# czbiohub-sf/yogo

Measured on AMD Instinct MI355X. Metric: training images/sec (772x1032 gray), higher is better.
Workload: dtype bf16; 1 GPU; BASELINE configs[2]: full train step (fwd+loss+bwd+clamp+AdamW), base_model, 772x1032x1 uint8, 7 classes; per_gpu_batch=128, global_batch=128, parallelism=dp1

## Files before the change

include/yogo_hip.h:

```cpp
#ifndef YOGO_HIP_H
#define YOGO_HIP_H

#include <stddef.h>

#ifdef __cplusplus
extern "C" {
#endif

typedef void* yogo_stream_t;

const char* yogo_hip_last_error(void);
int yogo_hip_abi_version(void);
int yogo_hip_launch_log(int enable);
int yogo_hip_launch_log_read(char* buf, size_t cap, size_t* needed);


int yogo_conv_packed_bytes(int Cin, int Cout, int ksize, int stride, int mode, size_t* bytes);
int yogo_conv_pack_f32(const float* w_oihw, float* packed, int Cin, int Cout, int ksize, int stride, int mode,
                       yogo_stream_t stream);
int yogo_conv2d_fwd_stats_shape(int B, int Cin, int Cout, int IH, int IW, int ksize, int stride, int* rows, int* mpad);
int yogo_conv2d_fwd_f32(const float* in, const float* packed, const float* bias, float* out, float* out_pre,
                        const float* chan_scale, float* stats_part, int B, int Cin, int Cout, int IH, int IW, int ksize,
                        int stride, int act, yogo_stream_t stream);
int yogo_conv2d_dgrad_f32(const float* dy, const float* packed_dgrad, float* dx, const float* act_ref, int ref_act,
// ... 45 lines not shown

int yogo_format_preds_workspace_bytes(int B, int Sy, int Sx, size_t* bytes);
int yogo_format_preds_batched(const float* pred, float* out_rows, long long* out_cells, int* out_count, void* workspace,
                              int B, int P, int Sy, int Sx, int cap, double obj_thresh, double iou_thresh, int box_format,
                              double min_class_confidence_threshold, yogo_stream_t stream);
int yogo_decode_format_preds_batched(const float* raw, const float* cxs, const float* cys, float* out_rows, long long* out_cells,
                                     int* out_count, void* workspace, int B, int P, int Sy, int Sx, int cap, float anchor_w,
                                     float anchor_h, float width_multiplier, float height_multiplier, int inference,
                                     double obj_thresh, double iou_thresh, int box_format, double min_class_confidence_threshold,
                                     yogo_stream_t stream);
int yogo_head1x1_decode_fwd_bf16(const void* x, const void* packed, const float* bias, float* out, const float* cxs, const float* cys,
                                 int B, int Cin, int P, int Sy, int Sx, float anchor_w, float anchor_h, float width_multiplier,
                                 float height_multiplier, int inference, yogo_stream_t stream);

int yogo_match_workspace_bytes(int B, int Sy, int Sx, int cap, size_t* bytes);
int yogo_match_preds_labels_batched(const float* rows, const int* counts, const float* labels, int* meta, int* pair_label,
                                    int* pair_pred, int* un_label, int* un_pred, float* lab_out, void* workspace, int B, int P, int Sy,
                                    int Sx, int cap, yogo_stream_t stream);
int yogo_match_gather(const float* rows, const float* lab_out, const int* meta, const int* pair_label, const int* pair_pred,
                      const int* un_label, const int* un_pred, float* preds, float* labels, float* missed, float* extra, int B, int P,
                      int cap, long long K, long long Km, long long Ke, yogo_stream_t stream);
int yogo_metrics_state_layout(int C, int T, int nbins, long long* offsets);
int yogo_metrics_accumulate(const float* rows, const float* lab_out, const int* meta, const int* pair_label, const int* pair_pred,
                            const int* un_label, const int* un_pred, const double* roc_thresholds, int T, const double* cal_edges,
                            int nbins, long long* acc, double* bin_conf, double* partial, float* map_rows, long long map_cap, int B,
                            int P, int cap, yogo_stream_t stream);

int yogo_pred_sink_state_layout(int C, long long* offsets);
int yogo_pred_sink_workspace_bytes(int B, size_t* bytes);
int yogo_pred_sink_append(const float* rows, const int* counts, int B, int cap, int P, int mode, int count_classes,
                          long long first_img_id, int img_h, int img_w, long long* state, float* arena, long long arena_cap,
                          int* img_counts, long long img_cap, void* workspace, yogo_stream_t stream);
int yogo_pred_text_bound(long long n_records, long long images, int P, size_t* text_bytes, size_t* workspace_bytes);
int yogo_pred_text_format(const float* records, long long n, int P, const int* img_counts, long long images, char* text,
                          long long text_cap, long long* img_offsets, long long* total, void* workspace, yogo_stream_t stream);

int yogo_bf16_channel_blocks(int C);
int yogo_conv_bf16_packed_bytes(int Cin, int Cout, int ksize, int mode, size_t* bytes);
int yogo_conv_bf16_pack(const float* w_oihw, const float* scale, void* packed, int Cin, int Cout, int ksize, int mode,
                        yogo_stream_t stream);
int yogo_conv2d_fwd_bf16_stats_shape(int B, int Cin, int Cout, int IH, int IW, int ksize, int stride, int* rows, int* mpad);
int yogo_conv2d_fwd_bf16(const void* in, const void* packed, const float* bias, void* out, float* out_f32,
                         const float* chan_scale, float* stats_part, int B, int Cin, int Cout, int IH, int IW, int ksize,
                         int stride, int act, yogo_stream_t stream);
int yogo_conv2d_fwd_bf16_pre(const void* in, const void* packed, const float* bias, void* out, void* out_pre,
                             const float* chan_scale, int B, int Cin, int Cout, int IH, int IW, int ksize, int stride, int act,
                             yogo_stream_t stream);
int yogo_conv_bf16_pack_blocks(int Cin, int Cout, int ksize, int mode, int* blocks);
int yogo_conv_bf16_pack_multi(const void* table, int n, int total_blocks, yogo_stream_t stream);
int yogo_bf16_signs_bytes(int B, int C, int H, int W, size_t* bytes);
int yogo_conv2d_fwd_bf16_signs(const void* in, const void* packed, const float* bias, void* out, void* signs,
                               const float* chan_scale, int B, int Cin, int Cout, int IH, int IW, int ksize, int stride, int act,
                               yogo_stream_t stream);
int yogo_conv2d_dgrad_bf16_signs(const void* dy, const void* packed_dgrad, void* dx, const void* signs,
                                 const float* chan_scale, int B, int Cin, int Cout, int IH, int IW, int ksize, int stride,
                                 yogo_stream_t stream);
int yogo_conv2d_dgrad_bf16(const void* dy, const void* packed_dgrad, void* dx, const void* act_ref, int ref_act,
                           const float* chan_scale, int B, int Cin, int Cout, int IH, int IW, int ksize, int stride,
                           yogo_stream_t stream);
int yogo_conv2d_wgrad_bf16in(const void* x, const void* g, float* dw, float* db, void* workspace, int B, int Cin, int Cout,
                             int IH, int IW, int ksize, int stride, float clip, yogo_stream_t stream);
int yogo_conv2d_wgrad_bf16_workspace_bytes(int B, int Cin, int Cout, int IH, int IW, int ksize, int stride, size_t* bytes);
int yogo_conv2d_wgrad_bf16(const void* x, const void* g, float* dw, float* db, void* workspace, int B, int Cin, int Cout,
                           int IH, int IW, int ksize, int stride, float clip, yogo_stream_t stream);
int yogo_wgrad_reduce_queue_create(void** queue_out);
int yogo_wgrad_reduce_queue_destroy(void* queue);
int yogo_wgrad_reduce_queue_reset(void* queue);
int yogo_wgrad_reduce_flush(void* queue, yogo_stream_t stream);
int yogo_conv2d_wgrad_bf16_deferred(const void* x, const void* g, float* dw, float* db, void* workspace, int B, int Cin, int Cout, int IH,
                                    int IW, int ks, int stride, float clip, void* queue, yogo_stream_t stream);
int yogo_conv_first_fwd_bf16(const void* in, int in_dtype, const float* w, const float* bias, void* out, int B, int Cin,
                             int Cout, int IH, int IW, int stride, int act, yogo_stream_t stream);
int yogo_conv_first_fwd_train_bf16(const void* in, int in_dtype, const float* w, const float* bias, void* out_bf16,
                                   const float* chan_scale, float* stats_part, int B, int Cin, int Cout, int IH, int IW,
                                   int stride, int act, yogo_stream_t stream);
int yogo_conv_first_wgrad_bf16g(const void* in, int in_dtype, const void* dy_bf16, float* part, int B, int Cin, int Cout,
                                int IH, int IW, int stride, yogo_stream_t stream);
int yogo_conv_first_bn_wgrad_cols(int Cin, int Cout, int* cols);
int yogo_conv_first_bn_wgrad_bf16(const void* in, int in_dtype, const void* g, const void* z, const float* mean,
                                  const float* invstd, const float* gamma, const float* beta, float* part, int B, int Cin,
                                  int Cout, int IH, int IW, int stride, int act, yogo_stream_t stream);
int yogo_conv_first_bn_wgrad_finalize(const float* sums, const float* mean, const float* invstd, const float* gamma,
                                      const float* w_oihw, float* dw, float* dgamma, float* dbeta, int B, int Cin, int Cout,
                                      int IH, int IW, int stride, int training, float clip, yogo_stream_t stream);
int yogo_bn_apply_act_bf16(const void* z, void* y, const float* mean, const float* invstd_or_var, int stat_is_var, float eps,
                           const float* gamma, const float* beta, int B, int C, int HW, int act, yogo_stream_t stream);
int yogo_bn_bwd_bf16_rows(int B, int HW, int* rows);
int yogo_bn_stats_bf16(const void* z, float* part, int B, int C, int HW, yogo_stream_t stream);
int yogo_bn_bwd_bf16(const void* g, const void* z, void* dz, const float* mean, const float* invstd, const float* gamma,
                     const float* beta, int act, float* dgamma, float* dbeta, float* part, float* sums, int B, int C, int HW,
                     int training, float clip, yogo_stream_t stream);
int yogo_bn_bwd_bf16_head(const void* gh, const float* head_w, int P, const void* z, void* dz, const float* mean, const float* invstd,
                          const float* gamma, const float* beta, int act, float* dgamma, float* dbeta, float* part, float* sums, int B,
                          int C, int HW, int training, float clip, yogo_stream_t stream);
int yogo_nchw_f32_to_bf16_8c(const float* in, void* out, int B, int C, int HW, yogo_stream_t stream);
int yogo_bf16_8c_to_nchw_f32(const void* in, float* out, int B, int C, int HW, yogo_stream_t stream);

int yogo_conv_first_mfma_supported(int in_dtype, int Cin, int Cout, int IH, int IW, int stride);
int yogo_conv_first_mfma_stats_rows(int B, int IH, int IW, int* rows);
int yogo_conv_first_mfma(const void* in, const float* w, const float* bias, void* z, void* y, const float* mean,
                         const float* invstd, const float* gamma, const float* beta, float* stats_part, int B, int Cout, int IH,
                         int IW, int act, yogo_stream_t stream);

int yogo_conv_first_gram_rows(int B, int IH, int IW, int* rows);
int yogo_conv_first_gram(const void* in, void* part, double* gram, float* gram_f32, int B, int IH, int IW, yogo_stream_t stream);
int yogo_bn_stats_from_gram(const double* gram, const float* w, const float* bias, int Cout, long long count, float eps,
// ... 91 lines not shown
```

yogo_amd/csrc/conv_bf16.hip:

```cpp
#include "conv_bf16_plan.h"
#include "conv_bf16_ws.h"
#include "conv_bf16_ws16.h"
#include "conv_bf16_ws3.h"
#include "plan_switches.h"

#ifdef YOGO_DIAG
static int g_diag_dbg = 0, g_diag_nodma = 0;
static unsigned long long* g_diag_stamps = nullptr;
static size_t g_diag_stamps_bytes = 0;
extern "C" int yogo_diag_conv_bf16(int dbg_bits, int no_dma, void* stamps, size_t stamps_bytes) {
  g_diag_dbg = dbg_bits; g_diag_nodma = no_dma;
  g_diag_stamps = reinterpret_cast<unsigned long long*>(stamps); g_diag_stamps_bytes = stamps_bytes;
  return YOGO_OK;
}
template <typename Q>
void bf_diag_persistent(Q* q, hipStream_t stream) {
  q->dbg = g_diag_dbg;
  q->stamps = (g_diag_stamps != nullptr && g_diag_stamps_bytes >= 512 * 128) ? g_diag_stamps : nullptr;
  if (q->stamps) (void)hipMemsetAsync(g_diag_stamps, 0, 512 * 128, stream);
}
#else
template <typename Q>
void bf_diag_persistent(Q*, hipStream_t) {}
#endif
// ... 183 lines not shown
  BfTiledPlan pl;
  if (int e = bf_plan_tiled(r, &pl)) return e;
  return launch_conv_bf16_tiled(r, pl, stream);
}

}

extern "C" int yogo_conv2d_fwd_bf16_stats_shape(int B, int Cin, int Cout, int IH, int IW, int ks, int stride, int* rows, int* mpad) {
  ConvBf16Request r;
  if (int e = bf_request(B, Cin, Cout, IH, IW, ks, stride, BF_FORWARD, &r)) return e;
  BfTiledPlan pl;
  if (int e = bf_plan_tiled(r, &pl)) return e;
  if (rows) *rows = pl.rows;
  if (mpad) *mpad = pl.mpad;
  return YOGO_OK;
}

extern "C" int yogo_conv2d_fwd_bf16(const void* in, const void* packed, const float* bias, void* out, float* out_f32,
                                    const float* chan_scale, float* stats_part, int B, int Cin, int Cout, int IH, int IW,
                                    int ks, int stride, int act, hipStream_t stream) {
  YOGO_CHECK_ARG(in && packed && (out || out_f32), "conv2d_fwd_bf16: null pointer");
  ConvBf16Request r;
  if (int e = bf_request(B, Cin, Cout, IH, IW, ks, stride, BF_FORWARD, &r)) return e;
  r.in = in; r.packed = packed; r.bias = bias; r.out = out; r.out_f32 = out_f32; r.chan_scale = chan_scale; r.stats_part = stats_part; r.act = act;
  return launch_conv_bf16(r, stream);
}

extern "C" int yogo_conv2d_fwd_bf16_pre(const void* in, const void* packed, const float* bias, void* out, void* out_pre,
                                        const float* chan_scale, int B, int Cin, int Cout, int IH, int IW, int ks, int stride,
                                        int act, hipStream_t stream) {
  YOGO_CHECK_ARG(in && packed && out && out_pre, "conv2d_fwd_bf16_pre: null pointer");
  ConvBf16Request r;
  if (int e = bf_request(B, Cin, Cout, IH, IW, ks, stride, BF_FORWARD, &r)) return e;
  r.in = in; r.packed = packed; r.bias = bias; r.out = out; r.out_pre = out_pre; r.chan_scale = chan_scale; r.act = act;
  return launch_conv_bf16(r, stream);
}

extern "C" int yogo_bf16_signs_bytes(int B, int C, int H, int W, size_t* bytes) {
  YOGO_CHECK_ARG(bytes && B >= 0 && C > 0 && H > 0 && W > 0, "bf16_signs_bytes: bad arguments");
  *bytes = (size_t)B * H * W * (bf_mpad_of(C) / 8);
  return YOGO_OK;
}

extern "C" int yogo_conv2d_fwd_bf16_signs(const void* in, const void* packed, const float* bias, void* out, void* signs,
                                          const float* chan_scale, int B, int Cin, int Cout, int IH, int IW, int ks, int stride,
                                          int act, hipStream_t stream) {
  YOGO_CHECK_ARG(in && packed && out && signs, "conv2d_fwd_bf16_signs: null pointer");
  ConvBf16Request r;
  if (int e = bf_request(B, Cin, Cout, IH, IW, ks, stride, BF_FORWARD, &r)) return e;
  r.in = in; r.packed = packed; r.bias = bias; r.out = out; r.signs = signs; r.chan_scale = chan_scale; r.act = act;
  return launch_conv_bf16(r, stream);
}

extern "C" int yogo_conv2d_dgrad_bf16_signs(const void* dy, const void* packed_dgrad, void* dx, const void* signs,
                                            const float* chan_scale, int B, int Cin, int Cout, int IH, int IW, int ks, int stride,
                                            hipStream_t stream) {
  YOGO_CHECK_ARG(dy && packed_dgrad && dx && signs, "conv2d_dgrad_bf16_signs: null pointer");
  ConvBf16Request r;
  if (int e = bf_request(B, Cin, Cout, IH, IW, ks, stride, BF_DGRAD, &r)) return e;
  r.in = dy; r.packed = packed_dgrad; r.out = dx; r.ref_act = ACT_LEAKY; r.signs = const_cast<void*>(signs); r.signs_read = true; r.chan_scale = chan_scale;
  return launch_conv_bf16(r, stream);
}

extern "C" int yogo_conv2d_dgrad_bf16(const void* dy, const void* packed_dgrad, void* dx, const void* act_ref, int ref_act,
                                      const float* chan_scale, int B, int Cin, int Cout, int IH, int IW, int ks, int stride,
                                      hipStream_t stream) {
  YOGO_CHECK_ARG(dy && packed_dgrad && dx, "conv2d_dgrad_bf16: null pointer");
  ConvBf16Request r;
  if (int e = bf_request(B, Cin, Cout, IH, IW, ks, stride, BF_DGRAD, &r)) return e;
  r.in = dy; r.packed = packed_dgrad; r.out = dx; r.act_ref = act_ref; r.ref_act = ref_act; r.chan_scale = chan_scale;
  return launch_conv_bf16(r, stream);
}
```

yogo_amd/csrc/conv_bf16_plan.h:

```cpp
#pragma once
#include "common.h"

#define BF_LDS_BUDGET (80 * 1024)
#define BF_LDS_MAX (160 * 1024)

__host__ __device__ inline int bf_pick_mw(int M) { return M <= 32 ? 1 : (M <= 64 ? 2 : 4); }
__host__ __device__ inline int bf_kb_of(int K) { return (K + 15) / 16 * 2; }
__host__ __device__ inline int bf_mpad_of(int M) { const int t = 32 * bf_pick_mw(M); return (M + t - 1) / t * t; }

struct ConvBf16Request {
  const void* in;
  const void* packed;
  const float* bias;
  void* out;
  float* out_f32;
  void* out_pre;
  const void* act_ref;
  int ref_act;
  void* signs;
  bool signs_read;
  const float* chan_scale;
  float* stats_part;
  int B, K, M, IH, IW, OH, OW, ks, a, s2d, act;
#ifdef YOGO_DIAG
  int dbg;
  unsigned long long* stamps;
  size_t stamps_bytes;
#endif
};

struct BfTiling {
  int ncb, TW, tiles_per_band, CKb, rows_max, LW, ldsw_off, lds_dummy, lds_bytes, dma, ni_slots, n_slots, bufu;
};

struct BfTiledPlan {
  int MW, NW, NWV, PF;
  bool wide64;
  BfTiling tl;
  bool ring;
  int lean4, rowdma, lwp;
  int dma;
  bool use_pp;
  int ni_slots, n_slots, ldsw_off, bufu, bufs, lds_bytes;
  dim3 grid;
  int rows, mpad;
};

int launch_conv_bf16_tiled(const ConvBf16Request& r, const BfTiledPlan& pl, hipStream_t stream);
bool conv_bf16_s2d_direct_eligible(int K, int M, int OH, int OW, int B);
int launch_conv_bf16_s2d_direct(const void* in, const void* packed, void* out, const void* signs, const float* chan_scale, int B, int K, int M, int IH, int IW,
                                int OH, int OW, hipStream_t stream);
bool conv_bf16_staged_eligible(int K, int M, int stride, int IH, int IW, int OH, int OW, int B);
int launch_conv_bf16_staged(const void* in, const void* packed, const float* bias, void* out, void* signs, const float* chan_scale, int B, int K, int M, int IH,
                            int IW, int OH, int OW, int stride, int act, hipStream_t stream);
bool conv_bf16_head_fwd_eligible(int K, int M, int plane, int B);
int launch_conv_bf16_head_fwd(const void* in, const void* packed, const float* bias, float* out_f32, int B, int K, int M, int plane, hipStream_t stream);
```

yogo_amd/csrc/plan_switches.h:

```cpp
#pragma once

bool plan_ws();
int plan_ws16_mode();
bool plan_direct();
bool plan_staged();
bool plan_head();
bool plan_first_bn_wgrad_pairs();
bool plan_first_mfma_pairs();
bool plan_tiled_pp();
bool plan_tiled_ring();
bool plan_tiled_lean4();
bool plan_tiled_rowdma();
```

yogo_amd/csrc/plan_switches.hip:

```cpp
#include "common.h"
#include "plan_switches.h"

#ifndef BF_WS16_MODE
#define BF_WS16_MODE 1
#endif
#ifdef BF_NO_ROWDMA
#define BF_ROWDMA_DEFAULT false
#else
#define BF_ROWDMA_DEFAULT true
#endif

#define PLAN_HOOK_SWITCHES(X)                                                              \
  X(bool, plan_ws, true, yogo_hook_conv_bf16_persistent)                                   \
  X(int, plan_ws16_mode, BF_WS16_MODE, yogo_hook_conv_bf16_ws16)                           \
  X(bool, plan_direct, true, yogo_hook_conv_bf16_direct)                                   \
  X(bool, plan_staged, true, yogo_hook_conv_bf16_staged)                                   \
  X(bool, plan_head, true, yogo_hook_conv_bf16_head)                                       \
  X(bool, plan_first_bn_wgrad_pairs, true, yogo_hook_conv_first_bn_wgrad_pairs)            \
  X(bool, plan_first_mfma_pairs, true, yogo_hook_conv_first_mfma_pairs)
#define PLAN_DIAG_SWITCHES(X)                                                              \
  X(bool, plan_tiled_pp, true, yogo_diag_conv_bf16_pp)                                     \
  X(bool, plan_tiled_ring, true, yogo_diag_conv_bf16_ring)                                 \
  X(bool, plan_tiled_lean4, true, yogo_diag_conv_bf16_lean4)                               \
  X(bool, plan_tiled_rowdma, BF_ROWDMA_DEFAULT, yogo_diag_conv_bf16_rowdma)

#define PLAN_CONSTANT(T, NAME, DEFAULT, SETTER) \
  T NAME() { return DEFAULT; }
#define PLAN_VARIABLE(T, NAME, DEFAULT, SETTER)                                            \
  static T g_##NAME = DEFAULT;                                                             \
  T NAME() { return g_##NAME; }                                                            \
  extern "C" int SETTER(int v) { g_##NAME = static_cast<T>(v); return YOGO_OK; }

#if defined(YOGO_TEST_HOOKS) || defined(YOGO_DIAG)
PLAN_HOOK_SWITCHES(PLAN_VARIABLE)
#else
PLAN_HOOK_SWITCHES(PLAN_CONSTANT)
#endif
#ifdef YOGO_DIAG
PLAN_DIAG_SWITCHES(PLAN_VARIABLE)
#else
PLAN_DIAG_SWITCHES(PLAN_CONSTANT)
#endif
```

yogo_amd/engine.py:

```python
from __future__ import annotations

import threading
import weakref
from dataclasses import dataclass, field
from typing import Dict, List, Optional, Tuple

import torch
from torch import nn

from yogo_amd import _hip

ACT_NONE, ACT_LEAKY, ACT_SILU = 0, 1, 2


@dataclass
class Layer:
    conv: nn.Conv2d
    bn: Optional[nn.BatchNorm2d] = None
    act: int = ACT_NONE
    drop: Optional[nn.Dropout2d] = None

    @property
    def cin(self) -> int:
        return self.conv.in_channels
# ... 272 lines not shown
                          IW, L.s, st)
                red = torch.empty(L.cout, nj, dtype=torch.float32, device=dev)
                _hip.call("yogo_partials_reduce", part, rows, L.cout * nj, clip, red, st)
                dw.copy_(red[:, : nj - 1].reshape(dw.shape))
                if has_bias:
                    db = dst(L.conv.bias)
                    db.copy_(red[:, nj - 1])
                    grads[id(L.conv.bias)] = db
            else:
                wsb = _hip.query_size("yogo_conv2d_wgrad_workspace_bytes", B, L.cin, L.cout, IH, IW, L.k, L.s)
                ws = torch.empty(wsb // 4, dtype=torch.float32, device=dev)
                db = dst(L.conv.bias) if has_bias else None
                self._tick("wgrad", i, 2.0 * B * L.cout * L.cin * L.k * L.k * OH * OW)
                _hip.call("yogo_conv2d_wgrad_f32", S.x_in, g, dw, db, ws, B, L.cin, L.cout, IH, IW, L.k, L.s, clip, st)
                self._tock()
                if has_bias:
                    grads[id(L.conv.bias)] = db
            grads[id(L.conv.weight)] = dw
            if on_layer is not None:
                on_layer(i)
            if i > 0:
                Lp, Sp = self.layers[i - 1], saved[i - 1]
                ref_act = Lp.act
                if Lp.bn is not None:
                    act_ref, ref_act = None, ACT_NONE
                elif Lp.act == ACT_SILU:
                    act_ref = Sp.pre
                    if act_ref is None:
                        raise RuntimeError("yogo_amd: missing saved pre-activation for a SiLU block")
                elif Lp.act == ACT_LEAKY:
                    act_ref = Sp.y
                else:
                    act_ref = None
                dx = torch.empty(B, L.cin, IH, IW, dtype=torch.float32, device=dev)
                pk = self._packed(i, 1)
                mw_tag = 20 if L.s == 2 else (4 if L.cin > 64 else (2 if L.cin > 32 else 1))
                self._tick("dgrad", i, 2.0 * B * L.cout * L.cin * L.k * L.k * OH * OW, mw=mw_tag)
                _hip.call("yogo_conv2d_dgrad_f32", g, pk, dx, act_ref, ref_act, Sp.mask, B, L.cin, L.cout, IH, IW, L.k, L.s, st)
                self._tock()
                g = dx
        bb = self.backbone_ref()
        return [grads.get(id(p)) for p in bb.parameters()]



def _blocks(c: int) -> int:
    return ((c + 15) // 16) * 2


_FUSE_LAYER0_BWD = True
_L0_NO_Z = True
_WGRAD_DEFER_REDUCE = True
_L01_FUSE_BWD = True
_HEAD_BN_FUSE = True


def _packed_bf16(eng: Engine, i: int, mode: int) -> torch.Tensor:
    L = eng.layers[i]
    w = L.conv.weight
    key = (i, 10 + mode)
    buf = _pack_hit(eng, key, w)
    if buf is not None:
        return buf
    nbytes = _hip.query_size("yogo_conv_bf16_packed_bytes", L.cin, L.cout, L.k, mode)
    buf = torch.empty(nbytes, dtype=torch.uint8, device=w.device)
    _hip.call("yogo_conv_bf16_pack", _f32(w.detach()), None, buf, L.cin, L.cout, L.k, mode, _hip.stream_ptr())
    eng._pack[key] = (w._version, w.data_ptr(), buf)
    return buf


def _pack_all_bf16(eng: Engine) -> None:
    jobs = [(i, mode) for i in range(1, len(eng.layers)) for mode in (0, 2 if (eng.layers[i].s == 2 and eng.layers[i].k == 3) else 1)]
    ws = [eng.layers[i].conv.weight for i, _ in jobs]
    if any(w.dtype != torch.float32 or not w.is_contiguous() for w in ws) or not jobs:
        return
    if all(_pack_hit(eng, (i, 10 + m), w) is not None for (i, m), w in zip(jobs, ws)):
        return
    dev = ws[0].device
    key = tuple(w.data_ptr() for w in ws)
    st = eng._pack_multi
    if st is None or st[0] != key:
        bufs, rows, blk = [], [], 0
        for (i, mode), w in zip(jobs, ws):
            L = eng.layers[i]
            buf = torch.empty(_hip.query_size("yogo_conv_bf16_packed_bytes", L.cin, L.cout, L.k, mode), dtype=torch.uint8, device=dev)
            bufs.append(buf)
            rows.append([w.data_ptr(), 0, buf.data_ptr(), L.cin, L.cout, L.k, mode, blk])
            blk += _hip.query_ints("yogo_conv_bf16_pack_blocks", 1, L.cin, L.cout, L.k, mode)[0]
        st = (key, bufs, torch.tensor(rows, dtype=torch.int64, device=dev), blk)
        eng._pack_multi = st
    _, bufs, table, blk = st
    _hip.call("yogo_conv_bf16_pack_multi", table, len(jobs), blk, _hip.stream_ptr())
    for (i, mode), w, buf in zip(jobs, ws, bufs):
        eng._pack[(i, 10 + mode)] = (w._version, w.data_ptr(), buf)


def _dropout_masks(eng: Engine, B: int, dev) -> Dict[int, torch.Tensor]:
    act = [(i, float(L.drop.p)) for i, L in enumerate(eng.layers) if L.drop is not None and L.drop.training and L.drop.p > 0]
    if not act:
        return {}
    key = (B, tuple(act), str(dev))
    cached = eng._drop_consts
    if cached is None or cached[0] != key:
        sizes = [B * eng.layers[i].cout for i, _ in act]
        pvec = torch.cat([torch.full((n,), p, dtype=torch.float32) for n, (_, p) in zip(sizes, act)]).to(dev)
        cached = (key, sizes, pvec, 1.0 / (1.0 - pvec))
# ... 58 lines not shown


def _layer_fwd_bf16(eng: Engine, i: int, L: Layer, S: Saved, bias, bn_train: bool, last: bool, B: int, H: int, W: int, st) -> torch.Tensor:
    cur, mask, dev = S.x_in, S.mask, S.x_in.device
    OH, OW = L.out_hw(H, W)
    has_bn = L.bn is not None
    if last and (has_bn or mask is not None):
        raise RuntimeError("yogo_amd: BatchNorm / Dropout on the last layer is not supported by the bf16 path")
    fused_act = ACT_NONE if has_bn else L.act
    out8 = None if last else torch.empty(B, _blocks(L.cout), OH, OW, 8, dtype=torch.bfloat16, device=dev)
    out32 = torch.empty(B, L.cout, OH, OW, dtype=torch.float32, device=dev) if last else None
    stats = None
    rows = mpad = 0
    if i == 0:
        if bn_train:
            rows, mpad = _hip.query_ints("yogo_conv_first_stats_rows", 1, B, H, W, L.s)[0], L.cout
            stats = torch.empty(rows * mpad * 2, dtype=torch.float32, device=dev)
        _hip.call("yogo_conv_first_fwd_train_bf16", cur, 0 if cur.dtype == torch.uint8 else 1, _f32(L.conv.weight.detach()), bias,
                  out8, mask, stats, B, L.cin, L.cout, H, W, L.s, fused_act, st)
    else:
        pk = _packed_bf16(eng, i, 0)
        nbytes = B * (_blocks(L.cin) * 8 * H * W * 2 + (L.cout * OH * OW * 4 if last else _blocks(L.cout) * 8 * OH * OW * 2))
        eng._tick("fwd", i, 2.0 * B * L.cout * L.cin * L.k * L.k * OH * OW, mw=34 if (L.cout > 64 and L.s == 1) else (35 if (L.cout > 64 and L.cin > 64 and L.k == 3) else 30), nbytes=nbytes)
        if L.act == ACT_SILU and not has_bn:
            S.pre = torch.empty_like(out8)
            _hip.call("yogo_conv2d_fwd_bf16_pre", cur, pk, bias, out8, S.pre, mask, B, L.cin, L.cout, H, W, L.k, L.s, fused_act, st)
        elif L.act == ACT_LEAKY and not has_bn and not last:
            S.signs = torch.empty(_hip.query_size("yogo_bf16_signs_bytes", B, L.cout, OH, OW), dtype=torch.uint8, device=dev)
            _hip.call("yogo_conv2d_fwd_bf16_signs", cur, pk, bias, out8, S.signs, mask, B, L.cin, L.cout, H, W, L.k, L.s, fused_act, st)
        else:
            _hip.call("yogo_conv2d_fwd_bf16", cur, pk, bias, out8, out32, mask, None, B, L.cin, L.cout, H, W, L.k, L.s, fused_act, st)
        eng._tock()
    if not has_bn:
        S.y = out32 if last else out8
        return S.y
    bn = L.bn
    gamma, beta = _bn_affine(L, dev)
    y = torch.empty_like(out8)
    if bn_train:
        if i > 0:
            rows, mpad = _hip.query_ints("yogo_bn_bwd_bf16_rows", 1, B, OH * OW)[0], L.cout
            stats = torch.empty(rows * mpad * 2, dtype=torch.float32, device=dev)
            _hip.call("yogo_bn_stats_bf16", out8, stats, B, L.cout, OH * OW, st)
        mean, invstd = _bn_finalize(eng, L, "yogo_bn_finalize", stats, rows, mpad, count=B * OH * OW, dev=dev, st=st)
    else:
        invstd = torch.empty(L.cout, dtype=torch.float32, device=dev)
        _hip.call("yogo_bn_invstd", bn.running_var, float(bn.eps), invstd, L.cout, st)
        mean = bn.running_mean
    _hip.call("yogo_bn_apply_act_bf16", out8, y, mean, invstd, 0, float(bn.eps), gamma, beta, B, L.cout, OH * OW, L.act, st)
    S.mean, S.invstd, S.bn_train, S.z, S.y = mean, invstd, bn_train, out8, y
    return y


def forward_bf16_train(eng: Engine, x: torch.Tensor) -> Tuple[torch.Tensor, List[Saved]]:
    _check_bf16_train_input(eng, x)
    dev, st, B = x.device, _hip.stream_ptr(), x.shape[0]
    _pack_all_bf16(eng)
    masks = _dropout_masks(eng, B, dev)
    cur = x.contiguous() if x.dtype == torch.uint8 else _f32(x)
    H, W = int(cur.shape[2]), int(cur.shape[3])
    saved: List[Saved] = []
    n = len(eng.layers)
    for i, L in enumerate(eng.layers):
        OH, OW = L.out_hw(H, W)
        if OH <= 0 or OW <= 0:
            raise RuntimeError(f"yogo_amd: image too small at layer {i}")
        last = i == n - 1
        has_bn = L.bn is not None
        if L.act == ACT_SILU and not has_bn and (i == 0 or last):
            raise RuntimeError("yogo_amd: bf16 training of a first / last SiLU block without BatchNorm is not implemented (use fp32)")
        bias = _f32(L.conv.bias.detach()) if L.conv.bias is not None else None
        S = Saved(x_in=cur, mask=masks.get(i))
        bn_train = has_bn and (L.bn.training or L.bn.running_mean is None)
        if (i == 0 and has_bn and S.mask is None and not last and cur.dtype == torch.uint8
                and _hip.lib().yogo_conv_first_mfma_supported(0, L.cin, L.cout, H, W, L.s)):
            cur = _first_mfma_fwd_bf16(eng, L, S, bias, bn_train, B, H, W, st)
        else:
            cur = _layer_fwd_bf16(eng, i, L, S, bias, bn_train, last, B, H, W, st)
        saved.append(S)
        H, W = OH, OW
    return cur, saved


def backward_bf16_train(eng: Engine, saved: List[Saved], graw: torch.Tensor,
                        grad_out: Optional[Dict[int, torch.Tensor]] = None, on_layer=None,
                        trace: Optional[dict] = None, flush_layers=None, stop_at: int = 0) -> List[Optional[torch.Tensor]]:
    n = len(eng.layers)
    if not 0 <= stop_at < n:
        raise ValueError(f"yogo_amd: stop_at {stop_at} is not a layer of this {n}-layer network")
    st, dev, clip = _hip.stream_ptr(), graw.device, float(eng.clip)
    grads: Dict[int, torch.Tensor] = {}

    def dst(param: torch.Tensor) -> torch.Tensor:
        if grad_out is not None and id(param) in grad_out:
            return grad_out[id(param)]
        return torch.empty(param.shape, dtype=torch.float32, device=dev)

    queued_ws: List[torch.Tensor] = []
    wq = _wgrad_queue() if (_WGRAD_DEFER_REDUCE and (on_layer is None or flush_layers is not None)) else None
    flush_at = frozenset(flush_layers) if flush_layers is not None else frozenset()
    if wq is not None:
        _hip.call("yogo_wgrad_reduce_queue_reset", wq)
    if graw.dtype == torch.bfloat16 and graw.ndim == 5:
        g = graw
        B = g.shape[0]
    else:
        graw = _f32(graw)
        B, P, Sy, Sx = graw.shape
        g = torch.empty(B, _blocks(P), Sy, Sx, 8, dtype=torch.bfloat16, device=dev)
        _hip.call("yogo_nchw_f32_to_bf16_8c", graw, g, B, P, Sy * Sx, st)

    def bn_backward(L, S, g, head_g, OH, OW):
        gamma, beta = _bn_affine(L, dev)
        dgamma, dbeta = _bn_grad_dst(L.bn, dst, grads, L.cout, dev)
        rows = _hip.query_ints("yogo_bn_bwd_bf16_rows", 1, B, OH * OW)[0]
        part = torch.empty(rows * L.cout * 2, dtype=torch.float32, device=dev)
        sums = torch.empty(2 * L.cout, dtype=torch.float32, device=dev)
        if head_g is not None:
            dz = torch.empty(B, _blocks(L.cout), OH, OW, 8, dtype=torch.bfloat16, device=dev)
            _hip.call("yogo_bn_bwd_bf16_head", *head_g, S.z, dz, S.mean, S.invstd, gamma, beta, L.act, dgamma, dbeta,
                      part, sums, B, L.cout, OH * OW, 1 if S.bn_train else 0, clip, st)
        else:
            dz = g
            _hip.call("yogo_bn_bwd_bf16", g, S.z, dz, S.mean, S.invstd, gamma, beta, L.act, dgamma, dbeta, part, sums, B, L.cout, OH * OW,
                      1 if S.bn_train else 0, clip, st)
        return dz
# ... 386 lines not shown
```

Before: 11170 images/s.

## Fuse consecutive 3x3 stride-1 and stride-2 leaky conv layers into one staged kernel

Adds a kernel that computes a 16->32 stride-1 3x3 conv and the following 32->64 stride-2 3x3 conv in one pass. The first layer's output tile is kept in LDS and consumed directly by the second conv, with halo rows carried between tiles. Both outputs and their sign masks are still written for backward. The forward pass in Python detects eligible layer pairs and dispatches the fused call. The aim is to avoid a separate launch and a global-memory re-read of the intermediate activation. The cost is heavy LDS use, some recomputation at tile edges, and a complex schedule.

```diff
diff --git a/include/yogo_hip.h b/include/yogo_hip.h
--- a/include/yogo_hip.h
+++ b/include/yogo_hip.h
@@ -121,6 +121,11 @@
 int yogo_conv2d_fwd_bf16_signs(const void* in, const void* packed, const float* bias, void* out, void* signs,
                                const float* chan_scale, int B, int Cin, int Cout, int IH, int IW, int ksize, int stride, int act,
                                yogo_stream_t stream);
+int yogo_conv2d_fwd_bf16_signs_pair_eligible(int B, int C0, int C1, int C2, int IH, int IW);
+int yogo_conv2d_fwd_bf16_signs_pair(const void* in, const void* packed1, const float* bias1, void* out1, void* signs1,
+                                    const float* scale1, const void* packed2, const float* bias2, void* out2, void* signs2,
+                                    const float* scale2, int B, int C0, int C1, int C2, int IH, int IW, int act,
+                                    yogo_stream_t stream);
 int yogo_conv2d_dgrad_bf16_signs(const void* dy, const void* packed_dgrad, void* dx, const void* signs,
                                  const float* chan_scale, int B, int Cin, int Cout, int IH, int IW, int ksize, int stride,
                                  yogo_stream_t stream);
diff --git a/yogo_amd/csrc/conv_bf16.hip b/yogo_amd/csrc/conv_bf16.hip
--- a/yogo_amd/csrc/conv_bf16.hip
+++ b/yogo_amd/csrc/conv_bf16.hip
@@ -259,6 +259,20 @@
   return launch_conv_bf16(r, stream);
 }
 
+extern "C" int yogo_conv2d_fwd_bf16_signs_pair_eligible(int B, int C0, int C1, int C2, int IH, int IW) {
+  return conv_bf16_staged_pair_eligible(C0, C1, C2, IH, IW, B) ? 1 : 0;
+}
+extern "C" int yogo_conv2d_fwd_bf16_signs_pair(const void* in, const void* packed1, const float* bias1, void* out1, void* signs1, const float* scale1,
+                                               const void* packed2, const float* bias2, void* out2, void* signs2, const float* scale2, int B, int C0,
+                                               int C1, int C2, int IH, int IW, int act, hipStream_t stream) {
+  YOGO_CHECK_ARG(in && packed1 && out1 && signs1 && packed2 && out2 && signs2, "conv2d_fwd_bf16_signs_pair: null pointer");
+  YOGO_CHECK_ARG(B >= 0 && C0 > 0 && C1 > 0 && C2 > 0 && IH > 0 && IW > 0, "conv2d_fwd_bf16_signs_pair: unsupported shape");
+  if (plan_staged_pair() && act == ACT_LEAKY && conv_bf16_staged_pair_eligible(C0, C1, C2, IH, IW, B))
+    return launch_conv_bf16_staged_pair(in, packed1, bias1, out1, signs1, scale1, packed2, bias2, out2, signs2, scale2, B, C1, C2, IH, IW, act, stream);
+  if (int e = yogo_conv2d_fwd_bf16_signs(in, packed1, bias1, out1, signs1, scale1, B, C0, C1, IH, IW, 3, 1, act, stream)) return e;
+  return yogo_conv2d_fwd_bf16_signs(out1, packed2, bias2, out2, signs2, scale2, B, C1, C2, IH, IW, 3, 2, act, stream);
+}
+
 extern "C" int yogo_conv2d_dgrad_bf16_signs(const void* dy, const void* packed_dgrad, void* dx, const void* signs,
                                             const float* chan_scale, int B, int Cin, int Cout, int IH, int IW, int ks, int stride,
                                             hipStream_t stream) {
diff --git a/yogo_amd/csrc/conv_bf16_plan.h b/yogo_amd/csrc/conv_bf16_plan.h
--- a/yogo_amd/csrc/conv_bf16_plan.h
+++ b/yogo_amd/csrc/conv_bf16_plan.h
@@ -53,5 +53,9 @@
 bool conv_bf16_staged_eligible(int K, int M, int stride, int IH, int IW, int OH, int OW, int B);
 int launch_conv_bf16_staged(const void* in, const void* packed, const float* bias, void* out, void* signs, const float* chan_scale, int B, int K, int M, int IH,
                             int IW, int OH, int OW, int stride, int act, hipStream_t stream);
+bool conv_bf16_staged_pair_eligible(int C0, int C1, int C2, int IH, int IW, int B);
+int launch_conv_bf16_staged_pair(const void* in, const void* packed1, const float* bias1, void* out1, void* signs1, const float* scale1, const void* packed2,
+                                 const float* bias2, void* out2, void* signs2, const float* scale2, int B, int C1, int C2, int IH, int IW, int act,
+                                 hipStream_t stream);
 bool conv_bf16_head_fwd_eligible(int K, int M, int plane, int B);
 int launch_conv_bf16_head_fwd(const void* in, const void* packed, const float* bias, float* out_f32, int B, int K, int M, int plane, hipStream_t stream);
diff --git a/yogo_amd/csrc/conv_bf16_staged_pair.hip b/yogo_amd/csrc/conv_bf16_staged_pair.hip
--- /dev/null
+++ b/yogo_amd/csrc/conv_bf16_staged_pair.hip
@@ -0,0 +1,386 @@
+#include "bf16_dev.h"
+#include "conv_bf16_plan.h"
+
+struct ConvPairParams {
+  const u32x4* in;
+  const u32x4* wp1;
+  const float* bias1;
+  u32x4* out1;
+  unsigned char* signs1;
+  const float* scale1;
+  const u32x4* wp2;
+  const float* bias2;
+  u32x4* out2;
+  unsigned char* signs2;
+  const float* scale2;
+  int B, M1, M2, Mb2, IH, IW, OH2, OW2, act;
+  int tiles_per_col, tiles_per_row, nstrip, nq, nunit, ntiles;
+  unsigned m_tpr, m_nq;
+};
+
+#define CP_TW 31
+#define CP_RUN 13
+#ifdef BF_PAIR_NO_SB
+#define CP_SCHED_BARRIER()
+#else
+#define CP_SCHED_BARRIER() __builtin_amdgcn_sched_barrier(0)
+#endif
+
+namespace {
+__device__ __forceinline__ void cp_dma16(i32x4 rs, unsigned lds_addr, int voff) {
+  unsigned keep;
+  rs = uniform4(rs); lds_addr = uniform(lds_addr);
+  asm volatile("s_mov_b32 %0, m0\n\ts_mov_b32 m0, %2\n\ts_nop 4\n\tbuffer_load_dwordx4 %1, %3, 0 offen lds\n\ts_mov_b32 m0, %0"
+               : "=&s"(keep)
+               : "v"(voff), "s"(lds_addr), "s"(rs)
+               : "memory");
+}
+__device__ __forceinline__ void cp_wait_dma() { asm volatile("s_waitcnt vmcnt(0)" ::: "memory"); }
+template <int N>
+__device__ __forceinline__ void cp_wait_dma_but() {
+  static_assert(N >= 0 && N < 64, "vmcnt");
+  asm volatile("s_waitcnt vmcnt(%0)" ::"n"(N) : "memory");
+}
+__device__ __forceinline__ void cp_reads_done() { asm volatile("s_waitcnt lgkmcnt(0)" ::: "memory"); }
+
+__device__ __forceinline__ u32x4 cp_epi_group(const f32x16& acc, int gp, const float* lds_b, const float* my_scale, int cl, bool leaky, unsigned* sign) {
+  const float4 bA = *reinterpret_cast<const float4*>(lds_b + cl), bB = *reinterpret_cast<const float4*>(lds_b + cl + 8);
+  const float4 sA = *reinterpret_cast<const float4*>(my_scale + cl), sB = *reinterpret_cast<const float4*>(my_scale + cl + 8);
+  const float ba[8] = {bA.x, bA.y, bA.z, bA.w, bB.x, bB.y, bB.z, bB.w};
+  const float sa[8] = {sA.x, sA.y, sA.z, sA.w, sB.x, sB.y, sB.z, sB.w};
+  float v[8];
+#pragma unroll
+  for (int i = 0; i < 8; ++i) v[i] = fmaf(acc[8 * gp + i], sa[i], ba[i] * sa[i]);
+  if (leaky) {
+#pragma unroll
+    for (int i = 0; i < 8; i += 2) {
+      const f32x2 sv = (f32x2){v[i], v[i + 1]} * (f32x2){LEAKY_SLOPE, LEAKY_SLOPE};
+      asm("v_max_f32 %0, %1, %2" : "=v"(v[i]) : "v"(v[i]), "v"(sv.x));
+      asm("v_max_f32 %0, %1, %2" : "=v"(v[i + 1]) : "v"(v[i + 1]), "v"(sv.y));
+    }
+  }
+  unsigned m = 0;
+#pragma unroll
+  for (int i = 7; i >= 0; --i) asm("v_cmp_lt_f32_e32 vcc, 0, %1\n\tv_addc_co_u32_e32 %0, vcc, %0, %0, vcc" : "+v"(m) : "v"(v[i]) : "vcc");
+  *sign = m;
+  bf16x8 ob;
+#pragma unroll
+  for (int i = 0; i < 8; ++i) ob[i] = (__bf16)v[i];
+  const u32x4 w = __builtin_bit_cast(u32x4, ob);
+  const auto r0 = __builtin_amdgcn_permlane32_swap(w.x, w.z, false, false);
+  const auto r1 = __builtin_amdgcn_permlane32_swap(w.y, w.w, false, false);
+  return u32x4{r0[0], r1[0], r0[1], r1[1]};
+}
+}
+
+template <int R2, int NWV>
+struct PairGeom {
+  static constexpr int PW = 33, ROWU = 66;
+  static constexpr int NR1 = 2 * R2 + 1;
+  static constexpr int NR0 = NR1 + 2;
+  static constexpr int TU0 = 2 * NR0 * ROWU;
+  static constexpr int NDMA = (TU0 + 63) / 64;
+  static constexpr int IMGU = NDMA * 64;
+  static constexpr int WVU = IMGU;
+  static constexpr int NSTORE = 2 * R2 * 2 * 3 + R2 * 5;
+  static constexpr int W1U = 9 * 2 * 32, W2U = 9 * 4 * 64;
+  static constexpr int OFF_W2 = W1U, OFF_B1 = OFF_W2 + W2U, OFF_B2 = OFF_B1 + 8, OFF_S = OFF_B2 + 16, OFF_T = OFF_S + NWV * 64;
+  static constexpr int LDS_BYTES = (OFF_T + NWV * WVU) * 16;
+  static_assert(NDMA <= 16, "y0 image too large");
+  static_assert(LDS_BYTES <= 160 * 1024, "LDS");
+};
+
+template <int R2, int NWV>
+__global__ __launch_bounds__(64 * NWV) void conv_bf16_staged_pair_kernel(const ConvPairParams p) {
+  extern __shared__ __attribute__((aligned(16))) u32x4 lds_u[];
+  using G = PairGeom<R2, NWV>;
+  constexpr int PW = G::PW, ROWU = G::ROWU, NR1 = G::NR1, NR0 = G::NR0, TU0 = G::TU0, NDMA = G::NDMA, NT = 64 * NWV;
+  const int tid = threadIdx.x, lane = tid & 63, l31 = lane & 31, half = lane >> 5;
+  const int wave = __builtin_amdgcn_readfirstlane(tid >> 6);
+  float* lds_b1 = reinterpret_cast<float*>(lds_u + G::OFF_B1);
+  float* lds_b2 = reinterpret_cast<float*>(lds_u + G::OFF_B2);
+  float* const scale0 = reinterpret_cast<float*>(lds_u + G::OFF_S) + wave * 256;
+  const unsigned scale0_addr = (unsigned)(G::OFF_S * 16 + wave * 1024);
+#pragma unroll
+  for (int w = 0; w < 2; ++w) {
+    scale0[w * 128 + lane] = lane < p.M1 ? 1.f : 0.f;
+    scale0[w * 128 + 64 + lane] = lane < p.M2 ? 1.f : 0.f;
+  }
+  for (int i = tid; i < G::W1U; i += NT) lds_u[i] = p.wp1[i];
+  for (int i = tid; i < G::W2U; i += NT) lds_u[G::OFF_W2 + i] = p.wp2[i];
+  for (int i = tid; i < 96; i += NT) {
+    if (i < 32) lds_b1[i] = (p.bias1 != nullptr && i < p.M1) ? p.bias1[i] : 0.f;
+    else lds_b2[i - 32] = (p.bias2 != nullptr && i - 32 < p.M2) ? p.bias2[i - 32] : 0.f;
+  }
+  __syncthreads();
+  const int IH = p.IH, IW = p.IW, OH2 = p.OH2, OW2 = p.OW2;
+  const int kcb = IH * IW * 16, plane1 = IH * IW, plane1_16 = plane1 * 16, plane2 = OH2 * OW2, plane2_16 = plane2 * 16;
+  const bool leaky = p.act == ACT_LEAKY;
+  u32x4* const img0 = lds_u + G::OFF_T + wave * G::WVU;
+  const unsigned img0_addr = (unsigned)((G::OFF_T + wave * G::WVU) * 16);
+  int rel[NDMA];
+  unsigned rc[NDMA];
+#pragma unroll
+  for (int i = 0; i < NDMA; ++i) {
+    const int u = i * 64 + lane;
+    const int kb = u / (NR0 * ROWU), rem = u - kb * (NR0 * ROWU);
+    const int r = rem / ROWU, col = rem - r * ROWU;
+    rel[i] = kb * kcb + (r * IW + col) * 16;
+    rc[i] = u < TU0 ? (unsigned)(r << 16 | col) : 0xFFFFFFFFu;
+  }
+  auto stage = [&](int b, int j, int oy0, int which, bool need0) {
+    const unsigned y0_addr = img0_addr;
+    const int iy0 = 2 * oy0 - 2, ix0 = 2 * CP_TW * j - 2;
+    const i32x4 rs_in = rsrc(p.in + (size_t)b * 2 * IH * IW, (unsigned)(2 * kcb));
+    const int base = (iy0 * IW + ix0) * 16;
+#pragma unroll
+    for (int i = 0; i < NDMA; ++i) {
+      const int r = (int)(rc[i] >> 16), c = (int)(rc[i] & 0xFFFFu);
+      const bool ok = ((unsigned)(iy0 + r) < (unsigned)IH) && ((unsigned)(ix0 + c) < (unsigned)IW) && (r > 0 || need0);
+      cp_dma16(rs_in, y0_addr + (unsigned)i * 1024u, ok ? rel[i] + base : (int)OOB);
+    }
+    if (p.scale1 != nullptr) dma_dword_uniform(rsrc(p.scale1 + (size_t)b * p.M1, (unsigned)(p.M1 * 4)), scale0_addr + (unsigned)(which * 512), lane * 4, 0u);
+    if (p.scale2 != nullptr) dma_dword_uniform(rsrc(p.scale2 + (size_t)b * p.M2, (unsigned)(p.M2 * 4)), scale0_addr + (unsigned)(which * 512 + 256), lane * 4, 0u);
+  };
+  struct Pos { int unit, b, j, ty, ty_end; };
+  const int xcd = blockIdx.x & 7, slot = blockIdx.x >> 3, nslot = gridDim.x >> 3;
+  const int u8 = (p.nunit + 7) >> 3, u_end = min(p.nunit, (xcd + 1) * u8);
+  auto open_unit = [&](int unit, Pos* q) {
+    for (; unit < u_end; unit += nslot) {
+      const int sg = udivm1(unit, p.nq, p.m_nq), run = unit - sg * p.nq;
+      const int strip = sg * NWV + wave;
+      if (strip >= p.nstrip) continue;
+      q->unit = unit;
+      q->b = udivm1(strip, p.tiles_per_row, p.m_tpr);
+      q->j = strip - q->b * p.tiles_per_row;
+      q->ty = run * CP_RUN;
+      q->ty_end = min(p.tiles_per_col, q->ty + CP_RUN);
+      return true;
+    }
+    return false;
+  };
+  int cur = 0;
+  u32x4 carry[2][2] = {};
+  cp_reads_done();
+  Pos at;
+  bool have = open_unit(xcd * u8 + slot, &at), first = true, started = false;
+  if (have) stage(at.b, at.j, at.ty * R2, 0, at.ty != 0);
+  for (; have; cur ^= 1) {
+    const int b = at.b, j = at.j, oy0 = at.ty * R2;
+    Pos nx = at;
+    bool have_n = true, first_n = false;
+    if (at.ty + 1 < at.ty_end) nx.ty = at.ty + 1;
+    else { have_n = open_unit(at.unit + nslot, &nx); first_n = true; }
+    const u32x4* y0img = img0;
+    u32x4* y1img = img0;
+    const float* my_scale1 = scale0 + cur * 128;
+    const float* my_scale2 = my_scale1 + 64;
+    if (!started) cp_wait_dma();
+    else cp_wait_dma_but<G::NSTORE>();
+    started = true;
+    const bool top = oy0 == 0, fresh = first && !top;
+    u32x4 hold[NR1][2];
+    u32x4 st0[NR1][2];
+    unsigned sg1[NR1][2];
+    int hold_iu[2];
+#pragma unroll
+    for (int bk = 0; bk < 2; ++bk) hold_iu[bk] = half * NR0 * ROWU + ((32 * bk + l31) & 1) * PW + ((32 * bk + l31) >> 1);
+    {
+      const u32x4* bt = y0img + half * NR0 * ROWU + l31;
+      const u32x4* wk = lds_u + half * 32 + l31;
+#pragma unroll
+      for (int r = 0; r < NR1; ++r) {
+        if (r == 0 && !fresh) {
+#pragma unroll
+          for (int bk = 0; bk < 2; ++bk) {
+            y1img[hold_iu[bk]] = top ? u32x4{0u, 0u, 0u, 0u} : carry[bk][0];
+            hold[0][bk] = top ? u32x4{0u, 0u, 0u, 0u} : carry[bk][1];
+          }
+          continue;
+        }
+        f32x16 acc[2];
+#pragma unroll
+        for (int bk = 0; bk < 2; ++bk)
+#pragma unroll
+          for (int q = 0; q < 16; ++q) acc[bk][q] = 0.f;
+#pragma unroll
+        for (int tp = 0; tp < 9; ++tp) {
+          const int ky = tp / 3, kx = tp % 3;
+          if (tp % 3 == 0) CP_SCHED_BARRIER();
+          const bf16x8 av = __builtin_bit_cast(bf16x8, wk[tp * 2 * 32]);
+#pragma unroll
+          for (int bk = 0; bk < 2; ++bk) {
+            const bf16x8 bv = __builtin_bit_cast(bf16x8, bt[(r + ky) * ROWU + 32 * bk + kx]);
+            acc[bk] = __builtin_amdgcn_mfma_f32_32x32x16_bf16(av, bv, acc[bk], 0, 0, 0);
+          }
+        }
+        CP_SCHED_BARRIER();
+        const int yy = 2 * oy0 - 1 + r;
+#pragma unroll
+        for (int bk = 0; bk < 2; ++bk) {
+          const int c = 32 * bk + l31, xx = 2 * CP_TW * j - 1 + c;
+          const bool inside = (unsigned)yy < (unsigned)IH && (unsigned)xx < (unsigned)IW;
+          const int iu = hold_iu[bk] + r * ROWU;
+          unsigned sg = 0;
+#pragma unroll
+          for (int gp = 0; gp < 2; ++gp) {
+            unsigned m;
+            const u32x4 st = cp_epi_group(acc[bk], gp, lds_b1, my_scale1, 16 * gp + 4 * half, leaky, &m);
+            sg |= m << (8 * gp);
+            const u32x4 unit = inside ? st : u32x4{0u, 0u, 0u, 0u};
+            if (gp == 0) { y1img[iu] = unit; st0[r][bk] = unit; }
+            else hold[r][bk] = unit;
+            if (r == NR1 - 1) carry[bk][gp] = unit;
+          }
+          sg1[r][bk] = sg;
+        }
+      }
+    }
+    f32x16 acc[R2][2];
+#pragma unroll
+    for (int rr = 0; rr < R2; ++rr)
+#pragma unroll
+      for (int mb = 0; mb < 2; ++mb)
+#pragma unroll
+        for (int q = 0; q < 16; ++q) acc[rr][mb][q] = 0.f;
+    {
+      const u32x4* bt = y1img + half * NR0 * ROWU + l31;
+      const u32x4* wk = lds_u + G::OFF_W2 + half * 64 + l31;
+#pragma unroll
+      for (int kc = 0; kc < 2; ++kc) {
+        if (kc == 1) {
+          __builtin_amdgcn_sched_barrier(0);
+#pragma unroll
+          for (int r = 0; r < NR1; ++r)
+#pragma unroll
+            for (int bk = 0; bk < 2; ++bk) y1img[hold_iu[bk] + r * ROWU] = hold[r][bk];
+        }
+#pragma unroll
+        for (int tp = 0; tp < 9; ++tp) {
+          const int ky = tp / 3, kx = tp % 3;
+          const int boff = ky * ROWU + (kx & 1) * PW + (kx >> 1);
+          if (tp % (R2 * 2 >= 4 ? 1 : 3) == 0) CP_SCHED_BARRIER();
+          bf16x8 av[2];
+#pragma unroll
+          for (int mb = 0; mb < 2; ++mb) av[mb] = __builtin_bit_cast(bf16x8, wk[(tp * 4 + 2 * kc) * 64 + 32 * mb]);
+#pragma unroll
+          for (int rr = 0; rr < R2; ++rr) {
+            const bf16x8 bv = __builtin_bit_cast(bf16x8, bt[boff + rr * 2 * ROWU]);
+#pragma unroll
+            for (int mb = 0; mb < 2; ++mb) acc[rr][mb] = __builtin_amdgcn_mfma_f32_32x32x16_bf16(av[mb], bv, acc[rr][mb], 0, 0, 0);
+          }
+        }
+      }
+    }
+    __builtin_amdgcn_sched_barrier(0);
+    if (have_n) {
+      cp_reads_done();
+      stage(nx.b, nx.j, nx.ty * R2, cur ^ 1, first_n && nx.ty != 0);
+    }
+    {
+      const auto rs_o = __builtin_amdgcn_make_buffer_rsrc((void*)(p.out1 + (size_t)b * 4 * plane1), (short)0, 4 * plane1_16, RSRC_WORD3);
+      const auto rs_s = __builtin_amdgcn_make_buffer_rsrc((void*)(p.signs1 + (size_t)b * plane1 * 4), (short)0, plane1 * 4, RSRC_WORD3);
+#pragma unroll
+      for (int r = 1; r < NR1; ++r)
+#pragma unroll
+        for (int bk = 0; bk < 2; ++bk) {
+          const int c = 32 * bk + l31, yy = 2 * oy0 - 1 + r, xx = 2 * CP_TW * j - 1 + c;
+          const bool own = (unsigned)yy < (unsigned)IH && (unsigned)xx < (unsigned)IW && c >= 1 && c <= 2 * CP_TW;
+          const int o = yy * IW + xx;
+          __builtin_amdgcn_raw_buffer_store_b128(st0[r][bk], rs_o, own ? o * 16 + half * plane1_16 : (int)OOB, 0, 2);
+          __builtin_amdgcn_raw_buffer_store_b128(hold[r][bk], rs_o, own ? o * 16 + (2 + half) * plane1_16 : (int)OOB, 0, 2);
+          __builtin_amdgcn_raw_buffer_store_b16((unsigned short)sg1[r][bk], rs_s, own ? (half * plane1 + o) * 2 : (int)OOB, 0, 0);
+        }
+    }
+    const auto rs_o = __builtin_amdgcn_make_buffer_rsrc((void*)(p.out2 + (size_t)b * p.Mb2 * plane2), (short)0, p.Mb2 * plane2_16, RSRC_WORD3);
+    const auto rs_s = __builtin_amdgcn_make_buffer_rsrc((void*)(p.signs2 + (size_t)b * plane2 * 8), (short)0, plane2 * 8, RSRC_WORD3);
+    const int ox0 = CP_TW * j;
+#pragma unroll
+    for (int rr = 0; rr < R2; ++rr) {
+      const bool ov = l31 < CP_TW && ox0 + l31 < OW2 && oy0 + rr < OH2;
+      const int o = (oy0 + rr) * OW2 + ox0 + l31;
+      unsigned sg = 0;
+#pragma unroll
+      for (int mb = 0; mb < 2; ++mb)
+#pragma unroll
+        for (int gp = 0; gp < 2; ++gp) {
+          unsigned m;
+          const u32x4 st = cp_epi_group(acc[rr][mb], gp, lds_b2, my_scale2, 32 * mb + 16 * gp + 4 * half, leaky, &m);
+          sg |= m << (8 * (2 * mb + gp));
+          const int cb = 4 * mb + 2 * gp + half;
+          __builtin_amdgcn_raw_buffer_store_b128(st, rs_o, (ov && cb < p.Mb2) ? o * 16 + cb * plane2_16 : (int)OOB, 0, 0);
+        }
+      __builtin_amdgcn_raw_buffer_store_b32(sg, rs_s, ov ? (half * plane2 + o) * 4 : (int)OOB, 0, 0);
+    }
+    at = nx; have = have_n; first = first_n;
+  }
+}
+
+static int cp_rows() {
+#ifdef BF_PAIR_R2
+  return BF_PAIR_R2;
+#else
+  return 1;
+#endif
+}
+
+bool conv_bf16_staged_pair_eligible(int C0, int C1, int C2, int IH, int IW, int B) {
+  if (C0 != 16 || C1 != 32 || C2 <= 32 || C2 > 64) return false;
+  if (IH < 1 || IW < 1 || B <= 0 || IH >= 32000 || IW >= 32768) return false;
+  const long long OH2 = (IH - 1) / 2 + 1, OW2 = (IW - 1) / 2 + 1;
+  const long long Mb2 = ((C2 + 15) / 16) * 2;
+  if (4ll * IH * IW * 16 >= (1ll << 31) || Mb2 * OH2 * OW2 * 16 >= (1ll << 31)) return false;
+  const long long tpr = (OW2 + CP_TW - 1) / CP_TW, nstrip = (long long)B * tpr;
+  const int R2 = cp_rows();
+  const long long tpc = (OH2 + R2 - 1) / R2, nq = (tpc + CP_RUN - 1) / CP_RUN;
+  const long long nunit = ((nstrip + 5) / 6 + 1) * nq;
+  if (nstrip + 8 >= (1ll << 31) || nunit >= (1ll << 31)) return false;
+  if (!magic_div_exact(nunit, (int)nq) || !magic_div_exact(nstrip + 8, (int)tpr)) return false;
+  return true;
+}
+
+namespace {
+template <int R2, int NWV>
+int cp_launch(ConvPairParams p, int n_cu, hipStream_t stream) {
+  using G = PairGeom<R2, NWV>;
+  p.tiles_per_col = cdiv(p.OH2, R2);
+  p.tiles_per_row = cdiv(p.OW2, CP_TW);
+  p.nstrip = p.B * p.tiles_per_row;
+  p.nq = cdiv(p.tiles_per_col, CP_RUN);
+  p.nunit = cdiv(p.nstrip, NWV) * p.nq;
+  p.ntiles = p.nstrip * p.tiles_per_col;
+  p.m_tpr = magic_u32(p.tiles_per_row); p.m_nq = magic_u32(p.nq);
+  constexpr int lds = G::LDS_BYTES;
+  const int per_cu = max(1, min(16 / NWV, (160 * 1024) / lds));
+  const int grid = 8 * max(1, min(cdiv(p.nunit, 8), per_cu * n_cu / 8));
+  const void* kernel = reinterpret_cast<const void*>(&conv_bf16_staged_pair_kernel<R2, NWV>);
+  if (int e = yogo_func_dynamic_lds(kernel, lds, "conv_bf16_staged_pair")) return e;
+  hipLaunchKernelGGL((conv_bf16_staged_pair_kernel<R2, NWV>), dim3(grid), dim3(64 * NWV), lds, stream, p);
+  if (yogo_launch_log_enabled())
+    yogo_launch_log("conv_bf16_staged_pair_kernel<%d, %d> | C1=%d C2=%d in=%dx%d out=%dx%d tiles=%d grid=%d lds=%d act=%d bias=%d,%d scale=%d,%d units=%d l1_mfma_factor=%.2f",
+                    R2, NWV, p.M1, p.M2, p.IH, p.IW, p.OH2, p.OW2, p.ntiles, grid, lds, p.act, p.bias1 != nullptr, p.bias2 != nullptr,
+                    p.scale1 != nullptr, p.scale2 != nullptr, p.nunit, (double)((2 * R2 * min(CP_RUN, p.tiles_per_col) + 1) * 64) / (2 * R2 * min(CP_RUN, p.tiles_per_col) * 2 * CP_TW));
+  return YOGO_OK;
+}
+}
+
+int launch_conv_bf16_staged_pair(const void* in, const void* packed1, const float* bias1, void* out1, void* signs1, const float* scale1, const void* packed2,
+                                 const float* bias2, void* out2, void* signs2, const float* scale2, int B, int C1, int C2, int IH, int IW, int act,
+                                 hipStream_t stream) {
+  int n_cu;
+  if (int e = yogo_device_cus("conv_bf16_staged_pair", &n_cu)) return e;
+  ConvPairParams p{};
+  p.in = reinterpret_cast<const u32x4*>(in);
+  p.wp1 = reinterpret_cast<const u32x4*>(packed1); p.bias1 = bias1; p.out1 = reinterpret_cast<u32x4*>(out1);
+  p.signs1 = reinterpret_cast<unsigned char*>(signs1); p.scale1 = scale1;
+  p.wp2 = reinterpret_cast<const u32x4*>(packed2); p.bias2 = bias2; p.out2 = reinterpret_cast<u32x4*>(out2);
+  p.signs2 = reinterpret_cast<unsigned char*>(signs2); p.scale2 = scale2;
+  p.B = B; p.M1 = C1; p.M2 = C2; p.Mb2 = ((C2 + 15) / 16) * 2; p.IH = IH; p.IW = IW; p.OH2 = (IH - 1) / 2 + 1; p.OW2 = (IW - 1) / 2 + 1; p.act = act;
+  if (B <= 0) return YOGO_OK;
+  int rc;
+  if (cp_rows() == 2) rc = cp_launch<2, 6>(p, n_cu, stream);
+  else rc = cp_launch<1, 8>(p, n_cu, stream);
+  if (rc != YOGO_OK) return rc;
+  YOGO_CHECK_LAUNCH("conv_bf16_staged_pair");
+  return YOGO_OK;
+}
diff --git a/yogo_amd/csrc/plan_switches.h b/yogo_amd/csrc/plan_switches.h
--- a/yogo_amd/csrc/plan_switches.h
+++ b/yogo_amd/csrc/plan_switches.h
@@ -4,6 +4,7 @@
 int plan_ws16_mode();
 bool plan_direct();
 bool plan_staged();
+bool plan_staged_pair();
 bool plan_head();
 bool plan_first_bn_wgrad_pairs();
 bool plan_first_mfma_pairs();
diff --git a/yogo_amd/csrc/plan_switches.hip b/yogo_amd/csrc/plan_switches.hip
--- a/yogo_amd/csrc/plan_switches.hip
+++ b/yogo_amd/csrc/plan_switches.hip
@@ -15,6 +15,7 @@
   X(int, plan_ws16_mode, BF_WS16_MODE, yogo_hook_conv_bf16_ws16)                           \
   X(bool, plan_direct, true, yogo_hook_conv_bf16_direct)                                   \
   X(bool, plan_staged, true, yogo_hook_conv_bf16_staged)                                   \
+  X(bool, plan_staged_pair, true, yogo_hook_conv_bf16_staged_pair)                         \
   X(bool, plan_head, true, yogo_hook_conv_bf16_head)                                       \
   X(bool, plan_first_bn_wgrad_pairs, true, yogo_hook_conv_first_bn_wgrad_pairs)            \
   X(bool, plan_first_mfma_pairs, true, yogo_hook_conv_first_mfma_pairs)
diff --git a/yogo_amd/engine.py b/yogo_amd/engine.py
--- a/yogo_amd/engine.py
+++ b/yogo_amd/engine.py
@@ -348,6 +348,7 @@
 _L0_NO_Z = True
 _WGRAD_DEFER_REDUCE = True
 _L01_FUSE_BWD = True
+_PAIR_FWD = True
 _HEAD_BN_FUSE = True
 
 
@@ -512,6 +513,37 @@
     return y
 
 
+def _pair_fwd_eligible(eng: Engine, i: int, B: int, H: int, W: int) -> bool:
+    if i < 1 or i + 2 >= len(eng.layers):
+        return False
+    La, Lb = eng.layers[i], eng.layers[i + 1]
+    if not all(L.k == 3 and L.bn is None and L.act == ACT_LEAKY for L in (La, Lb)) or La.s != 1 or Lb.s != 2:
+        return False
+    return bool(_hip.lib().yogo_conv2d_fwd_bf16_signs_pair_eligible(B, La.cin, La.cout, Lb.cout, H, W))
+
+
+def _pair_fwd_bf16(eng: Engine, i: int, Sa: Saved, Sb: Saved, B: int, H: int, W: int, st) -> torch.Tensor:
+    La, Lb = eng.layers[i], eng.layers[i + 1]
+    dev = Sa.x_in.device
+    OH, OW = Lb.out_hw(H, W)
+    bias_a = _f32(La.conv.bias.detach()) if La.conv.bias is not None else None
+    bias_b = _f32(Lb.conv.bias.detach()) if Lb.conv.bias is not None else None
+    pk_a, pk_b = _packed_bf16(eng, i, 0), _packed_bf16(eng, i + 1, 0)
+    y1 = torch.empty(B, _blocks(La.cout), H, W, 8, dtype=torch.bfloat16, device=dev)
+    y2 = torch.empty(B, _blocks(Lb.cout), OH, OW, 8, dtype=torch.bfloat16, device=dev)
+    Sa.signs = torch.empty(_hip.query_size("yogo_bf16_signs_bytes", B, La.cout, H, W), dtype=torch.uint8, device=dev)
+    Sb.signs = torch.empty(_hip.query_size("yogo_bf16_signs_bytes", B, Lb.cout, OH, OW), dtype=torch.uint8, device=dev)
+    flops = 2.0 * B * 9 * (La.cout * La.cin * H * W + Lb.cout * Lb.cin * OH * OW)
+    nbytes = B * 16 * ((_blocks(La.cin) + _blocks(La.cout)) * H * W + _blocks(Lb.cout) * OH * OW)
+    eng._tick("fwd", i, flops, mw=30, nbytes=nbytes)
+    _hip.call("yogo_conv2d_fwd_bf16_signs_pair", Sa.x_in, pk_a, bias_a, y1, Sa.signs, Sa.mask, pk_b, bias_b, y2, Sb.signs, Sb.mask,
+              B, La.cin, La.cout, Lb.cout, H, W, ACT_LEAKY, st)
+    eng._tock()
+    Sb.x_in = y1
+    Sa.y, Sb.y = y1, y2
+    return y2
+
+
 def forward_bf16_train(eng: Engine, x: torch.Tensor) -> Tuple[torch.Tensor, List[Saved]]:
     _check_bf16_train_input(eng, x)
     dev, st, B = x.device, _hip.stream_ptr(), x.shape[0]
@@ -521,7 +553,11 @@
     H, W = int(cur.shape[2]), int(cur.shape[3])
     saved: List[Saved] = []
     n = len(eng.layers)
+    paired = -1
     for i, L in enumerate(eng.layers):
+        if i == paired:
+            H, W = L.out_hw(H, W)
+            continue
         OH, OW = L.out_hw(H, W)
         if OH <= 0 or OW <= 0:
             raise RuntimeError(f"yogo_amd: image too small at layer {i}")
@@ -532,6 +568,16 @@
         bias = _f32(L.conv.bias.detach()) if L.conv.bias is not None else None
         S = Saved(x_in=cur, mask=masks.get(i))
         bn_train = has_bn and (L.bn.training or L.bn.running_mean is None)
+        if _PAIR_FWD and _pair_fwd_eligible(eng, i, B, H, W):
+            OH2, OW2 = eng.layers[i + 1].out_hw(OH, OW)
+            if OH2 <= 0 or OW2 <= 0:
+                raise RuntimeError(f"yogo_amd: image too small at layer {i + 1}")
+            S2 = Saved(x_in=None, mask=masks.get(i + 1))
+            cur = _pair_fwd_bf16(eng, i, S, S2, B, H, W, st)
+            saved += [S, S2]
+            paired = i + 1
+            H, W = OH, OW
+            continue
         if (i == 0 and has_bn and S.mask is None and not last and cur.dtype == torch.uint8
                 and _hip.lib().yogo_conv_first_mfma_supported(0, L.cin, L.cout, H, W, L.s)):
             cur = _first_mfma_fwd_bf16(eng, L, S, bias, bn_train, B, H, W, st)
```

Measured after the change: 11320 images/s (median of 6 runs). 1.3% higher.
